# ecml-peagnn/graph_recsys_benchmark

Hardware: AMD Instinct MI355X
Metric: BPR-scored edges/sec, PEAGAT MovieLens-25m, emb_dim=64, 9 metapaths (higher is better)
Workload: dtype f32; 1 GPU; ml25m_shaped PEAGAT forward+BPR: N=273744 nodes, 9 metapaths x 2 steps, 208376439 messages/step, emb 64 / hidden 64 / repr 16, batch 4096 triples; headline=True, parallelism=single

## Files before the change

graph_recsys_benchmark_amd/csrc/ablate.hip:

```cpp
#include <algorithm>

#include "model.h"
#include "score_common.h"

namespace pea {
namespace {

template <int G, int PREG>
__global__ __launch_bounds__(256) void fuse_ablate_kernel(int64_t N, int P, int R, const float *__restrict__ stack,
                                                          int64_t ld, const ChanCols col_of_channel,
                                                          const float *__restrict__ att, int mode,
                                                          float *__restrict__ out, float *__restrict__ out_att) {
    const int64_t item = (int64_t)blockIdx.x * (256 / G) + threadIdx.x / G;
    const int sl = threadIdx.x % G;
    const bool valid = item < N;
    const int64_t n = valid ? item : 0;
    const bool in_row = sl * 4 < R;
    const bool active = valid && in_row;
    const int c4 = in_row ? sl * 4 : 0;
    const float *row = stack + n * ld + c4;
    const float4 zero = make_float4(0.f, 0.f, 0.f, 0.f);
    const bool mean = mode == PEA_FUSE_MEAN;
    float *dst = out + n * R + c4;
    const int64_t variant_stride = N * (int64_t)R;

    if constexpr (PREG > 0) {
        float4 x[PREG];
        float lg[PREG];
#pragma unroll
        for (int p = 0; p < PREG; ++p) {
            x[p] = zero;
            lg[p] = 0.f;
            if (p < P) {
                x[p] = ld4(row + col_of_channel.c[p]);
                if (!mean) lg[p] = chan_logit<G>(x[p], ld4(att + p * R + c4), in_row);
            }
        }
        for (int v = 0; v <= P; ++v) {
            const int masked = v - 1;
            float m = -3.0e38f, s = 0.f;
            float4 acc = zero;
#pragma unroll
            for (int p = 0; p < PREG; ++p) {
                if (p < P) {
                    const bool off = p == masked;
                    const float4 xv = off ? zero : x[p];
                    if (mean) {
                        acc.x += xv.x; acc.y += xv.y; acc.z += xv.z; acc.w += xv.w;
                    } else {
                        softmax_step(off ? 0.f : lg[p], xv, m, s, acc);
                    }
                }
            }
            const float inv = mean ? 1.0f / (float)P : 1.0f / s;
            if (active)
                *reinterpret_cast<float4 *>(dst + (int64_t)v * variant_stride) =
                    make_float4(acc.x * inv, acc.y * inv, acc.z * inv, acc.w * inv);
            if (v == 0 && out_att && valid) {
#pragma unroll
                for (int p = 0; p < PREG; ++p)
                    if (p < P && p % G == sl) out_att[n * P + p] = mean ? inv : expf(lg[p] - m) * inv;
            }
        }
    } else {
        for (int v = 0; v <= P; ++v) {
            const int masked = v - 1;
            float m = -3.0e38f, s = 0.f;
            float4 acc = zero;
            for (int p = 0; p < P; ++p) {
                float4 xv = ld4(row + col_of_channel.c[p]);
                if (p == masked) xv = zero;
                if (mean) {
                    acc.x += xv.x; acc.y += xv.y; acc.z += xv.z; acc.w += xv.w;
                    continue;
                }
                softmax_step(chan_logit<G>(xv, ld4(att + p * R + c4), in_row), xv, m, s, acc);
            }
            const float inv = mean ? 1.0f / (float)P : 1.0f / s;
            if (active)
                *reinterpret_cast<float4 *>(dst + (int64_t)v * variant_stride) =
                    make_float4(acc.x * inv, acc.y * inv, acc.z * inv, acc.w * inv);
            if (v == 0 && out_att) {
                for (int p = 0; p < P; ++p) {
                    float w = inv;
                    if (!mean) w = expf(chan_logit<G>(ld4(row + col_of_channel.c[p]), ld4(att + p * R + c4), in_row) - m) * inv;
                    if (valid && p % G == sl) out_att[n * P + p] = w;
                }
            }
        }
    }
}

constexpr int kRegSmall = 4, kRegChannels = 16;

template <int G>
int launch_fuse_ablate_g(int64_t N, int P, int R, const float *stack, int64_t ld, const ChanCols &cols, const float *att,
                         int mode, float *out, float *out_att, hipStream_t stream) {
    const unsigned blocks = (unsigned)((N + (256 / G) - 1) / (256 / G));
    if (P <= kRegSmall)
        PEA_LAUNCH((fuse_ablate_kernel<G, kRegSmall>), dim3(blocks), dim3(256), 0, stream, N, P, R, stack, ld, cols, att, mode,
                   out, out_att);
    else if (P <= kRegChannels)
        PEA_LAUNCH((fuse_ablate_kernel<G, kRegChannels>), dim3(blocks), dim3(256), 0, stream, N, P, R, stack, ld, cols, att,
                   mode, out, out_att);
    else
        PEA_LAUNCH((fuse_ablate_kernel<G, 0>), dim3(blocks), dim3(256), 0, stream, N, P, R, stack, ld, cols, att, mode, out,
                   out_att);
    PEA_HIP(hipGetLastError());
    return PEA_OK;
}

}

int launch_fuse_ablate(int64_t N, int P, int R, const float *stack, int64_t ld, const ChanCols &col_of_channel,
                       const float *att, int mode, float *out_tables, float *out_att, hipStream_t stream) {
    PEA_REQUIRE(N > 0 && stack && out_tables, PEA_ERR_ARG, "fuse_ablate: null argument");
    PEA_REQUIRE(P > 0 && P <= kMaxChannels && R > 0 && R % 4 == 0 && R <= 256, PEA_ERR_ARG,
                "fuse_ablate: P=%d R=%d (P <= 64, R a multiple of 4 and <= 256)", P, R);
    PEA_REQUIRE(mode == PEA_FUSE_ATT || mode == PEA_FUSE_MEAN, PEA_ERR_ARG, "fuse_ablate: mode %d", mode);
    PEA_REQUIRE(mode == PEA_FUSE_MEAN || att != nullptr, PEA_ERR_ARG, "fuse_ablate: att is required for 'att' fusion");
    PEA_REQUIRE(ld % 4 == 0, PEA_ERR_ARG, "fuse_ablate: stack row stride must be a multiple of 4");
    ProfScope ps("fuse_ablate", stream, 4.0 * (double)N * R * (2.0 * P + 1.0));
    switch (lanes_for_r(R)) {
        case 1: return launch_fuse_ablate_g<1>(N, P, R, stack, ld, col_of_channel, att, mode, out_tables, out_att, stream);
        case 2: return launch_fuse_ablate_g<2>(N, P, R, stack, ld, col_of_channel, att, mode, out_tables, out_att, stream);
        case 4: return launch_fuse_ablate_g<4>(N, P, R, stack, ld, col_of_channel, att, mode, out_tables, out_att, stream);
        case 8: return launch_fuse_ablate_g<8>(N, P, R, stack, ld, col_of_channel, att, mode, out_tables, out_att, stream);
        case 16: return launch_fuse_ablate_g<16>(N, P, R, stack, ld, col_of_channel, att, mode, out_tables, out_att, stream);
        case 32: return launch_fuse_ablate_g<32>(N, P, R, stack, ld, col_of_channel, att, mode, out_tables, out_att, stream);
        default: return launch_fuse_ablate_g<64>(N, P, R, stack, ld, col_of_channel, att, mode, out_tables, out_att, stream);
    }
}

}

using namespace pea;

extern "C" int pea_fuse_ablate(int64_t num_nodes, int P, int R, const float *stack, int64_t ld_stack,
                               const int *col_of_channel_host, const float *att, int fuse_mode, float *out_tables,
                               float *out_att, void *stream) {
    PEA_REQUIRE(num_nodes > 0 && stack && out_tables && col_of_channel_host, PEA_ERR_ARG, "fuse_ablate: null argument");
    PEA_REQUIRE(P > 0 && P <= kMaxChannels, PEA_ERR_ARG, "fuse_ablate: P=%d (1..%d)", P, kMaxChannels);
    ChanCols cols{};
    for (int p = 0; p < P; ++p) {
        PEA_REQUIRE(col_of_channel_host[p] >= 0 && col_of_channel_host[p] % 4 == 0 && col_of_channel_host[p] + R <= ld_stack,
                    PEA_ERR_ARG, "fuse_ablate: channel %d column %d outside the stack row", p, col_of_channel_host[p]);
        cols.c[p] = col_of_channel_host[p];
    }
    return launch_fuse_ablate(num_nodes, P, R, stack, ld_stack, cols, att, fuse_mode, out_tables, out_att, (hipStream_t)stream);
}

extern "C" int pea_model_forward_ablate(pea_model *model, const float *const *params_host, const float *x, const float *att,
                                        void *workspace, size_t workspace_bytes, float *out_tables, float *out_att,
                                        void *stream) {
    PEA_REQUIRE(out_tables, PEA_ERR_ARG, "forward_ablate: null argument");
    PEA_REQUIRE(!model || model->plan->shard_world == 1, PEA_ERR_ARG, "forward_ablate: single GPU only (the plan is sharded)");
    PEA_TRY(check_forward_args("forward_ablate", model, params_host, x, workspace, workspace_bytes, -1, nullptr));
    PEA_REQUIRE(model->d.fuse_mode == PEA_FUSE_MEAN || att, PEA_ERR_ARG, "forward_ablate: att is required for 'att' fusion");
    const AblateOut abl{out_tables, out_att};
    ForwardCall c;
    c.model = model;
    c.params = params_host;
    c.x = x;
    c.ldx = model->d.emb_dim;
    c.att = att;
    c.wsf = aligned_ws(workspace);
    c.stream = (hipStream_t)stream;
    c.abl = &abl;
    return model_forward(c);
}
```

graph_recsys_benchmark_amd/csrc/common.h:

```cpp
#pragma once
#include <hip/hip_runtime.h>

#include <cstdarg>
#include <cstdint>
#include <cstdio>
#include <functional>
#include <string>
#include <vector>

#include "../../include/peahip.h"

namespace pea {

void set_error(const char *fmt, ...);
const char *get_error();

#define PEA_HIP(call)                                                                          \
    do {                                                                                       \
        hipError_t e_ = (call);                                                                \
        if (e_ != hipSuccess) {                                                                \
            pea::set_error("%s:%d: %s failed: %s", __FILE__, __LINE__, #call,                 \
                           hipGetErrorString(e_));                                             \
            return PEA_ERR_HIP;                                                                \
        }                                                                                      \
// ... 293 lines not shown
    int blk_start[kMaxMlp2Chan + 1];
    const float *x;
    const float *a0;
    float *t1;
    float *images;
    float *bias1, *att_src1, *att_dst1;
    float *r1;
    int64_t ld_r1;
    int64_t ldx, ld_a0, ld_t1;
    float *h0;
    int64_t ld_h0;
    Mlp2Chan c[kMaxMlp2Chan];
};
size_t mlp2_image_bytes(int kind, int emb, int hid);
bool mlp2_supported(int kind, int emb, int hid, int out);
int launch_mlp2_pack(const Mlp2Launch &L, hipStream_t stream);
int launch_mlp2(const Mlp2Launch &L, const int *rows, int64_t n_rows, hipStream_t stream);

constexpr int kMaxChannels = 64;
constexpr int kScatterMaxCols = 1024;
struct ChanCols {
    int c[kMaxChannels];
};
struct FuseSelect {
    const int64_t *ids = nullptr;
    int64_t id_stride = 1, n = 0;
    float *out = nullptr;
    int *err = nullptr;
    int rank = 0, world = 1, tile = 1;
};
int launch_fuse(int64_t N, int P, int R, const float *stack, int64_t ld, const ChanCols &col_of_channel,
                const float *att, int masked, int mode, const int *rows, int64_t n_rows, float *out,
                float *out_stack, hipStream_t stream, const FuseSelect *sel = nullptr);

int launch_fuse_ablate(int64_t N, int P, int R, const float *stack, int64_t ld, const ChanCols &col_of_channel,
                       const float *att, int mode, float *out_tables, float *out_att, hipStream_t stream);
struct AblateOut {
    float *tables = nullptr;
    float *att = nullptr;
};

struct ForwardCall {
    pea_model *model = nullptr;
    int stage = -1;
    int part = PEA_PART_ALL;
    const float *const *params = nullptr;
    const float *x = nullptr;
    int64_t ldx = 0;
    const float *att = nullptr;
    int masked = -1;
    float *wsf = nullptr;
    float *out_repr = nullptr, *out_stack = nullptr;
    float *out_x = nullptr;
    int64_t ld_out_x = 0;
    int relu_last = 0;
    hipStream_t stream = nullptr;
    bool training = false;
    const FuseSelect *sel = nullptr;
    const AblateOut *abl = nullptr;
// ... 9 lines not shown
```

graph_recsys_benchmark_amd/csrc/fuse_score.hip:

```cpp
#include <algorithm>
#include <mutex>

#include "score_common.h"

namespace pea {
namespace {

template <int G>
__global__ __launch_bounds__(256) void fuse_kernel(int64_t n_rows, const int *__restrict__ rows, int P, int R,
                                                   const float *__restrict__ stack, int64_t ld,
                                                   const ChanCols col_of_channel,
                                                   const float *__restrict__ att, int masked, int mode,
                                                   float *__restrict__ out, float *__restrict__ out_stack,
                                                   unsigned fuse_blocks, const FuseSelect sel, int64_t N) {
    const bool pick = blockIdx.x >= fuse_blocks;
    const int64_t item = (int64_t)(pick ? blockIdx.x - fuse_blocks : blockIdx.x) * (256 / G) + threadIdx.x / G;
    const int sl = threadIdx.x % G;
    bool valid = item < (pick ? sel.n : n_rows);
    int64_t n = 0;
    if (pick) {
        const int64_t id = valid ? sel.ids[item * sel.id_stride] : 0;
        const bool in_range = id >= 0 && id < N;
        if (valid && !in_range && sl == 0) atomicOr(sel.err, 1);
        const bool mine = in_range && (id / sel.tile) % sel.world == sel.rank;
        if (valid && !mine && sl * 4 < R) *reinterpret_cast<float4 *>(sel.out + item * R + sl * 4) = make_float4(0.f, 0.f, 0.f, 0.f);
        valid = valid && mine;
        n = valid ? id : 0;
        out_stack = nullptr;
    } else {
        n = valid ? (rows ? rows[item] : item) : 0;
    }
    float *dst_row = pick ? sel.out + item * R : (out ? out + n * R : nullptr);
    const bool active = valid && sl * 4 < R;
    const int c4 = sl * 4 < R ? sl * 4 : 0;
    float m = -3.0e38f, s = 0.f;
    float4 acc = make_float4(0.f, 0.f, 0.f, 0.f);
    for (int p = 0; p < P; ++p) {
        float4 x = ld4(stack + n * ld + col_of_channel.c[p] + c4);
        if (p == masked) x = make_float4(0.f, 0.f, 0.f, 0.f);
        if (out_stack && active) *reinterpret_cast<float4 *>(out_stack + (n * P + p) * R + c4) = x;
        if (mode == PEA_FUSE_MEAN) {
            acc.x += x.x; acc.y += x.y; acc.z += x.z; acc.w += x.w;
            continue;
        }
        softmax_step(chan_logit<G>(x, ld4(att + p * R + c4), sl * 4 < R), x, m, s, acc);
    }
    if (!active || !dst_row) return;
    const float inv = mode == PEA_FUSE_MEAN ? 1.0f / (float)P : 1.0f / s;
    *reinterpret_cast<float4 *>(dst_row + c4) = make_float4(acc.x * inv, acc.y * inv, acc.z * inv, acc.w * inv);
}

__global__ __launch_bounds__(256) void bpr_kernel(int64_t B, int R, int64_t N, const float *__restrict__ repr,
                                                  const int64_t *__restrict__ triples, int64_t stride,
                                                  const float *fc1_w, const float *fc1_b, const float *fc2_w,
                                                  const float *fc2_b, float *pos, float *neg, float *block_sums,
                                                  int *err) {
    stage_mlp(R, fc1_w, fc1_b, fc2_w);
    const float *w1 = smem, *b1 = smem + 2 * R * R, *w2 = b1 + R;
    __shared__ float red[256];
    const int64_t b = (int64_t)blockIdx.x * 256 + threadIdx.x;
    float term = 0.f;
// ... 78 lines not shown
    if (uidx >= U) return;
    const int64_t u = unids[uidx];
    if (u < 0 || u >= N) {
        if (lane == 0) atomicOr(err, 1);
        return;
    }
    const bool shared = cand_stride == 0;
    int64_t keep0 = -1, keep1 = -1;
    if (shared) {
        if (lane < C) keep0 = cand[uidx * C + lane];
        if (kWave + lane < C) keep1 = cand[uidx * C + kWave + lane];
    }
    const float b2 = fc2_b[0];
    for (int v = 0; v < V; ++v) {
        const int64_t *cv = cand + (int64_t)v * cand_stride + uidx * C;
        const MlpScorer score(tables + (int64_t)v * N * R, u, R, b2);
        rank_one_user(score, [&](int base, int c) { return shared && base == 0 ? keep0 : shared && base == kWave ? keep1 : cv[c]; },
                      C, N, lane, (int64_t)v * U + uidx, scores, rank, auc, loss, err);
    }
}

}

int launch_fuse(int64_t N, int P, int R, const float *stack, int64_t ld, const ChanCols &col_of_channel,
                const float *att, int masked, int mode, const int *rows, int64_t n_rows, float *out,
                float *out_stack, hipStream_t stream, const FuseSelect *sel_in) {
    PEA_REQUIRE(P > 0 && P <= kMaxChannels && R > 0 && R % 4 == 0 && R <= 256, PEA_ERR_ARG,
                "fuse: P=%d R=%d (P <= 64, R a multiple of 4 and <= 256)", P, R);
    PEA_REQUIRE(masked < P, PEA_ERR_ARG, "fuse: masked channel %d out of range (P=%d)", masked, P);
    PEA_REQUIRE(mode == PEA_FUSE_MEAN || att != nullptr, PEA_ERR_ARG, "fuse: att is required for 'att' fusion");
    PEA_REQUIRE(ld % 4 == 0, PEA_ERR_ARG, "fuse: stack row stride must be a multiple of 4");
    if (!rows) n_rows = N;
    FuseSelect sel;
    if (sel_in && sel_in->n > 0) {
        sel = *sel_in;
        PEA_REQUIRE(sel.ids && sel.out && sel.err && sel.world >= 1 && sel.tile >= 1 && out != nullptr, PEA_ERR_ARG,
                    "fuse: batch-row selection needs ids, an output, an error flag and the fused table");
    }
    if (n_rows <= 0 && sel.n <= 0) return PEA_OK;
    const int G = lanes_for_r(R);
    ProfScope ps("fuse", stream, 4.0 * (double)(n_rows + sel.n) * R * (P + 1));
    const unsigned fuse_blocks = (unsigned)((std::max<int64_t>(n_rows, 0) + (256 / G) - 1) / (256 / G));
    const unsigned blocks = fuse_blocks + (unsigned)((sel.n + (256 / G) - 1) / (256 / G));
#define PEA_FUSE_CASE(g)                                                                                       \
    case g:                                                                                                    \
        PEA_LAUNCH(fuse_kernel<g>, dim3(blocks), dim3(256), 0, stream, n_rows, rows, P, R, stack, ld, \
                           col_of_channel, att, masked, mode, out, out_stack, fuse_blocks, sel, N);            \
        break;
    switch (G) {
        PEA_FUSE_CASE(1)
        PEA_FUSE_CASE(2)
        PEA_FUSE_CASE(4)
        PEA_FUSE_CASE(8)
        PEA_FUSE_CASE(16)
        PEA_FUSE_CASE(32)
        default:
            PEA_LAUNCH(fuse_kernel<64>, dim3(blocks), dim3(256), 0, stream, n_rows, rows, P, R, stack, ld,
                               col_of_channel, att, masked, mode, out, out_stack, fuse_blocks, sel, N);
    }
#undef PEA_FUSE_CASE
    PEA_HIP(hipGetLastError());
    return PEA_OK;
}

}

using pea::set_error;
using pea::err_flag_for_current_device;
using pea::read_err_flag;

extern "C" size_t pea_bpr_workspace_bytes(int64_t B) {
    const int64_t blocks = (B + 255) / 256;
    return (size_t)(blocks + 1) * sizeof(float) + 16;
}

static int check_r(int R) {
    PEA_REQUIRE(R > 0 && R % 4 == 0 && R <= 64, PEA_ERR_ARG, "repr_dim %d must be a multiple of 4, <= 64", R);
    return PEA_OK;
}

int *pea::err_flag_for_current_device() {
// ... 95 lines not shown
    {
        pea::ProfScope ps("rank_eval_multi", stream, (double)V * U * C * (4.0 * R + 12.0));
        PEA_LAUNCH(pea::rank_multi_kernel, dim3((unsigned)((U + 3) / 4)), dim3(256), sh, stream, V, U, C, R, num_nodes, tables, unids,
                   cand, cand_variant_stride, fc1_w, fc1_b, fc2_w, fc2_b, scores, rank, auc, loss, err);
    }
    int rc = hipGetLastError() == hipSuccess ? PEA_OK : PEA_ERR_HIP;
    if (rc == PEA_OK) rc = read_err_flag(err, stream, "rank_eval_multi");
    return rc;
}

extern "C" int pea_fuse(int64_t num_nodes, int P, int R, const float *stack, int64_t ld_stack,
                        const int *col_of_channel_host, const float *att, int masked_channel, int fuse_mode, float *out,
                        void *stream) {
    PEA_REQUIRE(num_nodes > 0 && stack && out && col_of_channel_host, PEA_ERR_ARG, "fuse: null argument");
    PEA_REQUIRE(P > 0 && P <= pea::kMaxChannels, PEA_ERR_ARG, "fuse: P=%d (1..%d)", P, pea::kMaxChannels);
    PEA_REQUIRE(fuse_mode == PEA_FUSE_ATT || fuse_mode == PEA_FUSE_MEAN, PEA_ERR_ARG, "fuse: mode %d", fuse_mode);
    PEA_REQUIRE(masked_channel >= -1, PEA_ERR_ARG, "fuse: masked channel %d", masked_channel);
    pea::ChanCols cols{};
    for (int p = 0; p < P; ++p) {
        PEA_REQUIRE(col_of_channel_host[p] >= 0 && col_of_channel_host[p] % 4 == 0 && col_of_channel_host[p] + R <= ld_stack,
                    PEA_ERR_ARG, "fuse: channel %d column %d outside the stack row", p, col_of_channel_host[p]);
        cols.c[p] = col_of_channel_host[p];
    }
    return pea::launch_fuse(num_nodes, P, R, stack, ld_stack, cols, att, masked_channel, fuse_mode, nullptr, num_nodes, out,
                            nullptr, (hipStream_t)stream);
}
```

graph_recsys_benchmark_amd/csrc/mlp2.hip:

```cpp
#include "common.h"

namespace pea {
namespace {

typedef float f32x16 __attribute__((ext_vector_type(16)));

__host__ __device__ inline int mlp2_image_floats(int ET, int HT) { return HT * ET * 256 + HT * 1024 + 2 * HT * 16; }

__global__ __launch_bounds__(256) void mlp2_pack_kernel(const Mlp2Launch L) {
    const int kPackSplit = (int)gridDim.x / L.n;
    const int chan = (int)blockIdx.x / kPackSplit, part = (int)blockIdx.x % kPackSplit;
    const Mlp2Chan &C = L.c[chan];
    const int EMB = L.emb, HID = L.hid, OUT = L.out;
    const int ET = EMB / 8, HT = HID / 32;
    const int t0 = part * 256 + (int)threadIdx.x, ts = 256 * kPackSplit;
    if (L.kind == PEA_KIND_SAGE) {
        const int KT = 2 * ET;
        float *img = L.images + (size_t)chan * mlp2_image_floats(KT, HT);
        float *wt0 = img, *wt1 = img + HT * KT * 256, *b0p = wt1 + HT * 1024;
        for (int idx = t0; idx < HT * KT * 256; idx += ts) {
            const int e = idx & 3, lane = (idx >> 2) & 63, qq = (idx >> 8) % KT, t = (idx >> 8) / KT;
            const int i = 32 * t + (lane & 31), k = 4 * (2 * (qq % ET) + (lane >> 5)) + e;
            wt0[idx] = (qq < ET ? C.w0 : C.w0_root)[(size_t)i * EMB + k];
        }
// ... 12 lines not shown
    float *img = L.images + (size_t)chan * mlp2_image_floats(ET, HT);
    float *wt0 = img, *wt1 = img + HT * ET * 256, *b0p = wt1 + HT * 1024;
    const bool gat = L.kind == PEA_KIND_GAT;
    const int EJ = EMB / 16, HJ = HID / 16;
    for (int idx = t0; idx < HJ * EJ * 256; idx += ts) {
        const int e = idx & 3, lane = (idx >> 2) & 63, j = (idx >> 8) % EJ, t = (idx >> 8) / EJ;
        const int i = 16 * t + (lane & 15), k = 16 * j + 4 * (lane >> 4) + e;
        wt0[idx] = gat ? C.w0[(size_t)i * EMB + k] : C.w0[(size_t)k * HID + i];
    }
    for (int idx = t0; idx < 2 * HJ * 256; idx += ts) {
        const int v = idx & 3, lane = (idx >> 2) & 63, t = (idx >> 8) % HJ, u = (idx >> 8) / HJ;
        const int o = 16 * u + (lane & 15), i = 16 * t + 4 * (lane >> 4) + v;
        wt1[idx] = o < OUT ? (gat ? C.w1[(size_t)o * HID + i] : C.w1[(size_t)i * OUT + o]) : 0.f;
    }
    for (int i = t0; i < HID; i += ts) b0p[i] = C.b0 ? C.b0[i] : 0.f;
    for (int o = t0; o < OUT; o += ts) {
        L.bias1[C.t1_col + o] = C.b1 ? C.b1[o] : 0.f;
        if (gat) {
            L.att_src1[C.t1_col + o] = C.att_src1[o];
            L.att_dst1[C.t1_col + o] = C.att_dst1[o];
        }
    }
    if (gat) {
        for (int k = (int)threadIdx.x * kPackSplit + part; k < EMB; k += ts) {
            float s = 0.f, d = 0.f;
            for (int i = 0; i < HID; ++i) {
                const float w = C.w0[(size_t)i * EMB + k];
                s = fmaf(C.att_src0[i], w, s);
                d = fmaf(C.att_dst0[i], w, d);
            }
            C.ws[k] = s;
            C.wd[k] = d;
        }
    }
}

extern __shared__ float mlp2_lds[];
template <int ET, int HT>
struct Mlp2Cfg {
    static constexpr int kThreads = (ET == 8 && HT == 2) ? 1024 : 512;
};

template <int ET>
struct Mlp2In {
    float4 xa[2][ET / 2];
    float sc[2];
    int row[2];
    bool valid[2];
};

template <int ET>
__device__ __forceinline__ void mlp2_load(const Mlp2Launch &L, const int *rows, int64_t n_rows, int64_t tile, int ch, int n16,
// ... 400 lines not shown
```

graph_recsys_benchmark_amd/csrc/model.hip:

```cpp
#include <algorithm>
#include <cstdlib>
#include <cstring>

#include "agg_build.h"

namespace pea {
namespace {

int pad4(int v) { return (v + 3) & ~3; }
int pad_ld(int v) { return (v + 31) & ~31; }
size_t pad_off(size_t v) { return (v + 63) & ~(size_t)63; }

int width_out(const pea_model_desc &d, int S, int s, int *heads_out) {
    const bool last = s == S - 1;
    int heads = d.kind == PEA_KIND_GAT ? d.heads : 1;
    if (S > 1 && last) heads = 1;
    *heads_out = heads;
    return last ? d.repr_dim : d.hidden_size;
}

int slots_of(const pea_model *m, int rel) {
    int n = m->plan->rels[(size_t)rel].n_slots;
    if (m->backward && rel < (int)m->reverse_of.size() && m->reverse_of[(size_t)rel] >= 0)
        n = std::max(n, m->plan->rels[(size_t)m->reverse_of[(size_t)rel]].n_slots);
// ... 334 lines not shown
    if (m->backward) {
        PEA_REQUIRE(desc->reverse_of != nullptr, PEA_ERR_ARG, "model: enable_backward needs reverse_of (relation -> reversed relation)");
        m->reverse_of.assign(desc->reverse_of, desc->reverse_of + plan->rels.size());
    }
    m->d.steps = nullptr;
    m->d.relation_of = nullptr;
    m->d.reverse_of = nullptr;
    m->n_slots_per_layer = desc->kind == PEA_KIND_GAT ? 4 : desc->kind == PEA_KIND_GCN ? 2 : 3;
    return build_schedule(m);
}

struct Fwd {
    const ForwardCall &c;
    pea_model *m;
    pea_plan *plan;
    float *pack;
    float *X;
    int64_t ldX;
    float *partial;
    bool sharded;
    const int *own_rows;
    int64_t n_own;
    bool hot_on;

    explicit Fwd(const ForwardCall &call)
        : c(call), m(call.model), plan(const_cast<pea_plan *>(call.model->plan)), pack(call.wsf),
          X(call.out_x ? call.out_x : call.wsf + call.model->off_x), ldX(call.out_x ? call.ld_out_x : call.model->ld_x),
          partial(call.wsf + call.model->off_partial), sharded(plan->shard_world > 1),
          own_rows(sharded ? plan->owned_rows : nullptr), n_own(sharded ? plan->n_owned : plan->N) {
        const char *hot_env = getenv("PEA_HOT");
        hot_on = hot_env && atoi(hot_env) != 0;
    }
    const float *param(const Unit &u, int slot) const {
        return c.params[(size_t)(m->chan_first[(size_t)u.p] + u.s) * (size_t)m->n_slots_per_layer + (size_t)slot];
    }
    bool self_loops() const { return (plan->flags & PEA_PLAN_SELF_LOOPS) != 0; }
};

struct LevelIO {
    Level &L;
    float *T, *O;
    const float *In;
    int ldIn;
    LevelOut out;
};
LevelIO level_io(const Fwd &f, int s) {
    pea_model *m = f.m;
    Level &L = m->levels[(size_t)s];
    float *O = f.c.wsf + L.off_o;
    return LevelIO{L,
                   f.c.wsf + L.off_t,
                   O,
                   s == 0 ? f.c.x : f.c.wsf + m->levels[(size_t)s - 1].off_o,
                   s == 0 ? (int)f.c.ldx : m->levels[(size_t)s - 1].ld_o,
// ... 64 lines not shown
        a.hot_K = hv->K;
        a.hot_frac = R.e_kept > 0 ? (double)hv->hot_edges / (double)R.e_kept : 0.0;
    }
    return PEA_OK;
}

AggMode forward_mode(int kind) { return kind == PEA_KIND_GAT ? AGG_GAT : kind == PEA_KIND_GCN ? AGG_GCN : AGG_MEAN; }

int aggregate_level(const Fwd &f, int s, AggMode mode) {
    const pea_model *m = f.m;
    pea_plan *plan = f.plan;
    const pea_model_desc &d = m->d;
    const bool training = f.c.training;
    float *wsf = f.c.wsf;
    const LevelIO io = level_io(f, s);
    const Level &L = io.L;
    const bool via_slots = f.sharded && s > 0;
    const bool mean2 = mode == AGG_MEAN && m->sage2;
    std::vector<AggGroup> gs;
    for (const GroupPlan &g : L.groups) {
        Relation &R = plan->rels[(size_t)g.rel];
        if (via_slots) PEA_REQUIRE(R.col_slot != nullptr, PEA_ERR_ARG, "relation %d has no exchange layout (pea_plan_set_sources)", g.rel);
        AggGroup a = agg_over(R);
        const bool skip0 = mode != AGG_MEAN && !g.last && f.self_loops() && !training;
        const bool skip0_mean = mean2 && !g.last && !training;
        if (skip0 || skip0_mean) skip_edgeless(a, R);
        if (training && mode == AGG_GAT) {
            a.stats = wsf + L.off_stats + 2 * g.a_k;
            a.ld_stats = L.ld_stats;
        }
        a.W = g.W;
        a.F = g.F;
        a.partial = f.partial + g.partial_off;
        a.neg_slope = d.negative_slope;
        set_traffic(a, R, mode != AGG_MEAN && f.self_loops() ? 1.0 : 0.0, mode == AGG_MEAN ? 1.0 : (double)g.n_convs,
                    table_rows(R, plan, via_slots));
        const Dest out = io.out.at(g.last, g.out_col);
        if (mode == AGG_MEAN && !mean2) {
            a.feat = io.In + g.col;
            a.ld_feat = io.ldIn;
            a.out = io.T + g.out_col;
            a.ld_out = L.ld_t;
        } else {
            a.feat = io.T + g.col;
            a.ld_feat = L.ld_t;
            a.out = out.ptr;
            a.ld_out = out.ld;
// ... 130 lines not shown
        GemmJob J = gemm_job(io.In, io.ldIn, f.m->d.emb_dim, f.pack + L.b_off + c_beg, L.ldb, c_end - c_beg, c_end - c_beg,
                             io.T + c_beg, L.ld_t);
        J.no_narrow = 1;
        J.rows = R.need_rows;
        J.n_rows = R.n_need;
        jobs.push_back(J);
        i = j;
    }
    root_jobs(f, 0, jobs);
    return launch_gemm_batch(jobs.data(), (int)jobs.size(), nullptr, 0, f.c.stream);
}

int transform_units(const Fwd &f, int s) {
    const LevelIO io = level_io(f, s);
    std::vector<GemmJob> jobs;
    for (const Unit &u : io.L.units) {
        GemmJob J = gemm_job(io.In + u.in_col, io.ldIn, u.in_w, f.pack + u.b_off, u.ldb, u.ldb, u.HF, io.T + u.t_col, io.L.ld_t);
        if (f.m->sage2 && !f.c.training) relu_on_load(f, s, u, J);
        if (f.self_loops() && !f.c.training) PEA_TRY(conv_on_load(f, s, u, J));
        jobs.push_back(J);
    }
    root_jobs(f, s, jobs);
    return launch_gemm_batch(jobs.data(), (int)jobs.size(), f.own_rows, f.n_own, f.c.stream);
}

int transform_level(const Fwd &f, int s) {
    if (f.m->d.kind == PEA_KIND_SAGE && !f.m->sage2) return transform_mean_first(f, s);
    if (!f.m->levels[(size_t)s].shared_input) return transform_units(f, s);
    return f.sharded ? transform_shared_sharded(f) : transform_shared(f);
}


int set_exchange(const Fwd &f, const Unit &u1, Mlp2Chan &C) {
    C.x_slot = nullptr;
    C.x_buf = nullptr;
    C.x_ld = 0;
    if (!f.sharded) return PEA_OK;
    for (const GroupPlan &g : f.m->levels[1].groups) {
        if (u1.t_col < g.col || u1.t_col >= g.col + g.W) continue;
        const Relation &R2 = f.plan->rels[(size_t)g.rel];
        PEA_REQUIRE(R2.slot_of_node != nullptr && g.xch_ld > 0, PEA_ERR_ARG,
                    "relation %d has no exchange layout (pea_plan_set_sources)", g.rel);
        C.x_slot = R2.slot_of_node;
        C.x_buf = f.c.wsf + g.xch_off + (u1.t_col - g.col);
        C.x_ld = g.xch_ld;
        return PEA_OK;
// ... 137 lines not shown
    const pea_model_desc &d = m->d;
    const int n_levels = (int)m->levels.size();
    const Fwd f(c);
    if (f.sharded) PEA_REQUIRE(f.plan->owned_rows != nullptr || f.plan->n_owned == 0, PEA_ERR_ARG, "sharded plan without owned rows");
    const int s_beg = c.stage < 0 ? 0 : c.stage, s_end = c.stage < 0 ? n_levels : c.stage + 1;
    PEA_REQUIRE(s_beg >= 0 && s_end <= n_levels, PEA_ERR_ARG, "forward: stage %d of %d", c.stage, n_levels);
    PEA_REQUIRE(c.part == PEA_PART_ALL || (f.sharded && c.stage >= 0), PEA_ERR_ARG, "forward: parts are stages of a sharded plan");
    const bool splits = m->fused2 && !c.training;
    const bool two_step = (m->fused2 && !c.training) || (m->fused2_train && c.training);
    const bool mean_first = d.kind == PEA_KIND_SAGE && !m->sage2;
    const AggMode mode = forward_mode(d.kind);
    for (int k = s_beg; k < s_end; ++k) {
        if (c.part == PEA_PART_REST && !(splits && k == 0)) continue;
        if (two_step) {
            PEA_TRY(k == 0 ? two_step_stage0(f) : aggregate_level(f, k, mode));
        } else {
            if (k == 0) PEA_TRY(pack_weights(f));
            if (k == 0 && !mean_first) PEA_TRY(transform_level(f, 0));
            PEA_TRY(aggregate_level(f, k, mode));
            if (mean_first) PEA_TRY(transform_level(f, k));
            else if (k + 1 < n_levels) PEA_TRY(transform_level(f, k + 1));
        }
        if (k != n_levels - 1) continue;
        if (c.abl)
            PEA_TRY(launch_fuse_ablate(f.plan->N, d.num_channels, d.repr_dim, f.X, f.ldX, m->x_col, c.att, d.fuse_mode, c.abl->tables,
                                       c.abl->att, c.stream));
        else if (c.out_repr || c.out_stack)
            PEA_TRY(launch_fuse(f.plan->N, d.num_channels, d.repr_dim, f.X, f.ldX, m->x_col, c.att, c.masked, d.fuse_mode, f.own_rows,
                                f.n_own, c.out_repr, c.out_stack, c.stream, c.sel));
    }
    return PEA_OK;
}

int check_forward_args(const char *who, const pea_model *model, const float *const *params, const float *x,
                       const void *workspace, size_t workspace_bytes, int masked, const int *stage) {
    PEA_REQUIRE(model && params && x && workspace, PEA_ERR_ARG, "%s: null argument", who);
    const int n_stages = (int)model->levels.size();
    if (stage) PEA_REQUIRE(*stage >= 0 && *stage < n_stages, PEA_ERR_ARG, "%s: stage %d of %d", who, *stage, n_stages);
    PEA_REQUIRE(workspace_bytes >= pea_model_workspace_bytes(model), PEA_ERR_NOMEM, "%s: workspace %zu < %zu bytes", who,
                workspace_bytes, pea_model_workspace_bytes(model));
    PEA_REQUIRE(masked >= -1 && masked < model->d.num_channels, PEA_ERR_ARG, "%s: masked channel %d", who, masked);
    return PEA_OK;
}

}

using namespace pea;

extern "C" int pea_model_create(const pea_plan *plan, const pea_model_desc *desc, pea_model **out) {
    PEA_REQUIRE(out != nullptr, PEA_ERR_ARG, "model: out is null");
    *out = nullptr;
    pea_model *m = new pea_model();
// ... 219 lines not shown
```

graph_recsys_benchmark_amd/csrc/score_common.h:

```cpp
#ifndef PEA_SCORE_COMMON_H_
#define PEA_SCORE_COMMON_H_

#include "common.h"

namespace pea {

int *err_flag_for_current_device();
int read_err_flag(int *err_dev, hipStream_t stream, const char *what);

inline int lanes_for_r(int R) {
    int g = 1;
    while (g * 4 < R) g <<= 1;
    return g;
}

namespace {

__device__ __forceinline__ float mlp_score(const float *__restrict__ ur, const float *__restrict__ ir, int R,
                                           const float *w1, const float *b1, const float *w2, float b2) {
    float o = 0.f;
    for (int k = 0; k < R; ++k) {
        const float *w = w1 + k * 2 * R;
        float a = 0.f;
        for (int c = 0; c < R; c += 4) {
            const float4 u = ld4(ur + c), wu = ld4(w + c);
            a += (u.x * wu.x + u.y * wu.y) + (u.z * wu.z + u.w * wu.w);
// ... 27 lines not shown
            a += (v[c].x * wi.x + v[c].y * wi.y) + (v[c].z * wi.z + v[c].w * wi.w);
        }
        a += b1[k];
        o = fmaf(fmaxf(a, 0.f), w2[k], o);
    }
    return o + b2;
}

template <int R4>
__device__ __forceinline__ void load_row(const float *p, float4 (&r)[R4]) {
#pragma unroll
    for (int c = 0; c < R4; ++c) r[c] = ld4(p + 4 * c);
}

extern __shared__ float smem[];

__device__ __forceinline__ void stage_mlp(int R, const float *fc1_w, const float *fc1_b, const float *fc2_w) {
    for (int i = threadIdx.x; i < 2 * R * R; i += blockDim.x) smem[i] = fc1_w[i];
    for (int i = threadIdx.x; i < R; i += blockDim.x) {
        smem[2 * R * R + i] = fc1_b[i];
        smem[2 * R * R + R + i] = fc2_w[i];
    }
    __syncthreads();
}

__device__ __forceinline__ float log_sigmoid_ref(float d) {
    return logf(1.0f / (1.0f + expf(-d)));
}

struct MlpScorer {
    const float *repr, *w1, *b1, *w2;
    float b2;
    int R;
    int64_t u;
    float4 ur[4];
    __device__ __forceinline__ MlpScorer(const float *repr_, int64_t u_, int R_, float b2_)
        : repr(repr_), w1(smem), b1(smem + 2 * R_ * R_), w2(smem + 2 * R_ * R_ + R_), b2(b2_), R(R_), u(u_) {
        if (R == 16) load_row<4>(repr + u * R, ur);
    }
    __device__ __forceinline__ float operator()(int64_t i) const {
        if (R == 16) {
            float4 ir[4];
            load_row<4>(repr + i * R, ir);
            return mlp_score_reg<4>(ur, ir, w1, b1, w2, b2);
        }
        return mlp_score(repr + u * R, repr + i * R, R, w1, b1, w2, b2);
// ... 66 lines not shown
```

Baseline: 129.7 billion edges/s.

## Defer edgeless-node last-layer rows to fuse kernel via self-loop copy path

For inference forwards that end in a fuse or ablate step, the last aggregation level now also skips edgeless (degree-zero) nodes. Their output is rebuilt inside the fuse kernels from the transformed row, bias, attention or GCN normalisation, and ReLU, with bias and attention vectors staged in LDS. This avoids a separate aggregation pass over those rows at the cost of more per-channel work and branching in the fuse kernels and extra LDS use. The GAT weight-folding loop in mlp2 is also unrolled into batched loads.

```diff
diff --git a/graph_recsys_benchmark_amd/csrc/ablate.hip b/graph_recsys_benchmark_amd/csrc/ablate.hip
--- a/graph_recsys_benchmark_amd/csrc/ablate.hip
+++ b/graph_recsys_benchmark_amd/csrc/ablate.hip
@@ -8,7 +8,7 @@
 
 template <int G, int PREG>
 __global__ __launch_bounds__(256) void fuse_ablate_kernel(int64_t N, int P, int R, const float *__restrict__ stack,
-                                                          int64_t ld, const ChanCols col_of_channel,
+                                                          int64_t ld, const ChanCols col_of_channel, const ChanCopy copy,
                                                           const float *__restrict__ att, int mode,
                                                           float *__restrict__ out, float *__restrict__ out_att) {
     const int64_t item = (int64_t)blockIdx.x * (256 / G) + threadIdx.x / G;
@@ -18,11 +18,13 @@
     const bool in_row = sl * 4 < R;
     const bool active = valid && in_row;
     const int c4 = in_row ? sl * 4 : 0;
-    const float *row = stack + n * ld + c4;
+    const float *row0 = stack + n * ld;
     const float4 zero = make_float4(0.f, 0.f, 0.f, 0.f);
     const bool mean = mode == PEA_FUSE_MEAN;
     float *dst = out + n * R + c4;
     const int64_t variant_stride = N * (int64_t)R;
+    const unsigned long long lone = copy_row_bits(copy, P, n);
+    stage_copy_rows(copy, P, R, smem);
 
     if constexpr (PREG > 0) {
         float4 x[PREG];
@@ -32,7 +34,7 @@
             x[p] = zero;
             lg[p] = 0.f;
             if (p < P) {
-                x[p] = ld4(row + col_of_channel.c[p]);
+                x[p] = chan_value(row0 + col_of_channel.c[p], copy.c[p], copy, smem + 3 * p * R, R, (lone >> p) & 1, n, c4, sl);
                 if (!mean) lg[p] = chan_logit<G>(x[p], ld4(att + p * R + c4), in_row);
             }
         }
@@ -68,7 +70,7 @@
             float m = -3.0e38f, s = 0.f;
             float4 acc = zero;
             for (int p = 0; p < P; ++p) {
-                float4 xv = ld4(row + col_of_channel.c[p]);
+                float4 xv = chan_value(row0 + col_of_channel.c[p], copy.c[p], copy, smem + 3 * p * R, R, (lone >> p) & 1, n, c4, sl);
                 if (p == masked) xv = zero;
                 if (mean) {
                     acc.x += xv.x; acc.y += xv.y; acc.z += xv.z; acc.w += xv.w;
@@ -83,7 +85,7 @@
             if (v == 0 && out_att) {
                 for (int p = 0; p < P; ++p) {
                     float w = inv;
-                    if (!mean) w = expf(chan_logit<G>(ld4(row + col_of_channel.c[p]), ld4(att + p * R + c4), in_row) - m) * inv;
+                    if (!mean) w = expf(chan_logit<G>(chan_value(row0 + col_of_channel.c[p], copy.c[p], copy, smem + 3 * p * R, R, (lone >> p) & 1, n, c4, sl), ld4(att + p * R + c4), in_row) - m) * inv;
                     if (valid && p % G == sl) out_att[n * P + p] = w;
                 }
             }
@@ -94,18 +96,18 @@
 constexpr int kRegSmall = 4, kRegChannels = 16;
 
 template <int G>
-int launch_fuse_ablate_g(int64_t N, int P, int R, const float *stack, int64_t ld, const ChanCols &cols, const float *att,
+int launch_fuse_ablate_g(int64_t N, int P, int R, const float *stack, int64_t ld, const ChanCols &cols, const ChanCopy &copy, const float *att,
                          int mode, float *out, float *out_att, hipStream_t stream) {
     const unsigned blocks = (unsigned)((N + (256 / G) - 1) / (256 / G));
     if (P <= kRegSmall)
-        PEA_LAUNCH((fuse_ablate_kernel<G, kRegSmall>), dim3(blocks), dim3(256), 0, stream, N, P, R, stack, ld, cols, att, mode,
-                   out, out_att);
+        PEA_LAUNCH((fuse_ablate_kernel<G, kRegSmall>), dim3(blocks), dim3(256), copy_lds_bytes(copy, P, R), stream, N, P, R, stack, ld, cols, copy, att,
+                   mode, out, out_att);
     else if (P <= kRegChannels)
-        PEA_LAUNCH((fuse_ablate_kernel<G, kRegChannels>), dim3(blocks), dim3(256), 0, stream, N, P, R, stack, ld, cols, att,
+        PEA_LAUNCH((fuse_ablate_kernel<G, kRegChannels>), dim3(blocks), dim3(256), copy_lds_bytes(copy, P, R), stream, N, P, R, stack, ld, cols, copy, att,
                    mode, out, out_att);
     else
-        PEA_LAUNCH((fuse_ablate_kernel<G, 0>), dim3(blocks), dim3(256), 0, stream, N, P, R, stack, ld, cols, att, mode, out,
-                   out_att);
+        PEA_LAUNCH((fuse_ablate_kernel<G, 0>), dim3(blocks), dim3(256), copy_lds_bytes(copy, P, R), stream, N, P, R, stack, ld, cols, copy, att, mode,
+                   out, out_att);
     PEA_HIP(hipGetLastError());
     return PEA_OK;
 }
@@ -113,22 +115,23 @@
 }
 
 int launch_fuse_ablate(int64_t N, int P, int R, const float *stack, int64_t ld, const ChanCols &col_of_channel,
-                       const float *att, int mode, float *out_tables, float *out_att, hipStream_t stream) {
+                       const ChanCopy &copy, const float *att, int mode, float *out_tables, float *out_att, hipStream_t stream) {
     PEA_REQUIRE(N > 0 && stack && out_tables, PEA_ERR_ARG, "fuse_ablate: null argument");
     PEA_REQUIRE(P > 0 && P <= kMaxChannels && R > 0 && R % 4 == 0 && R <= 256, PEA_ERR_ARG,
                 "fuse_ablate: P=%d R=%d (P <= 64, R a multiple of 4 and <= 256)", P, R);
     PEA_REQUIRE(mode == PEA_FUSE_ATT || mode == PEA_FUSE_MEAN, PEA_ERR_ARG, "fuse_ablate: mode %d", mode);
     PEA_REQUIRE(mode == PEA_FUSE_MEAN || att != nullptr, PEA_ERR_ARG, "fuse_ablate: att is required for 'att' fusion");
     PEA_REQUIRE(ld % 4 == 0, PEA_ERR_ARG, "fuse_ablate: stack row stride must be a multiple of 4");
+    PEA_REQUIRE(copy_lds_bytes(copy, P, R) <= kCopyLdsMax, PEA_ERR_ARG, "fuse_ablate: copy rows of a %d x %d stack", P, R);
     ProfScope ps("fuse_ablate", stream, 4.0 * (double)N * R * (2.0 * P + 1.0));
     switch (lanes_for_r(R)) {
-        case 1: return launch_fuse_ablate_g<1>(N, P, R, stack, ld, col_of_channel, att, mode, out_tables, out_att, stream);
-        case 2: return launch_fuse_ablate_g<2>(N, P, R, stack, ld, col_of_channel, att, mode, out_tables, out_att, stream);
-        case 4: return launch_fuse_ablate_g<4>(N, P, R, stack, ld, col_of_channel, att, mode, out_tables, out_att, stream);
-        case 8: return launch_fuse_ablate_g<8>(N, P, R, stack, ld, col_of_channel, att, mode, out_tables, out_att, stream);
-        case 16: return launch_fuse_ablate_g<16>(N, P, R, stack, ld, col_of_channel, att, mode, out_tables, out_att, stream);
-        case 32: return launch_fuse_ablate_g<32>(N, P, R, stack, ld, col_of_channel, att, mode, out_tables, out_att, stream);
-        default: return launch_fuse_ablate_g<64>(N, P, R, stack, ld, col_of_channel, att, mode, out_tables, out_att, stream);
+        case 1: return launch_fuse_ablate_g<1>(N, P, R, stack, ld, col_of_channel, copy, att, mode, out_tables, out_att, stream);
+        case 2: return launch_fuse_ablate_g<2>(N, P, R, stack, ld, col_of_channel, copy, att, mode, out_tables, out_att, stream);
+        case 4: return launch_fuse_ablate_g<4>(N, P, R, stack, ld, col_of_channel, copy, att, mode, out_tables, out_att, stream);
+        case 8: return launch_fuse_ablate_g<8>(N, P, R, stack, ld, col_of_channel, copy, att, mode, out_tables, out_att, stream);
+        case 16: return launch_fuse_ablate_g<16>(N, P, R, stack, ld, col_of_channel, copy, att, mode, out_tables, out_att, stream);
+        case 32: return launch_fuse_ablate_g<32>(N, P, R, stack, ld, col_of_channel, copy, att, mode, out_tables, out_att, stream);
+        default: return launch_fuse_ablate_g<64>(N, P, R, stack, ld, col_of_channel, copy, att, mode, out_tables, out_att, stream);
     }
 }
 
@@ -147,7 +150,7 @@
                     PEA_ERR_ARG, "fuse_ablate: channel %d column %d outside the stack row", p, col_of_channel_host[p]);
         cols.c[p] = col_of_channel_host[p];
     }
-    return launch_fuse_ablate(num_nodes, P, R, stack, ld_stack, cols, att, fuse_mode, out_tables, out_att, (hipStream_t)stream);
+    return launch_fuse_ablate(num_nodes, P, R, stack, ld_stack, cols, ChanCopy{}, att, fuse_mode, out_tables, out_att, (hipStream_t)stream);
 }
 
 extern "C" int pea_model_forward_ablate(pea_model *model, const float *const *params_host, const float *x, const float *att,
diff --git a/graph_recsys_benchmark_amd/csrc/common.h b/graph_recsys_benchmark_amd/csrc/common.h
--- a/graph_recsys_benchmark_amd/csrc/common.h
+++ b/graph_recsys_benchmark_amd/csrc/common.h
@@ -339,6 +339,23 @@
 struct ChanCols {
     int c[kMaxChannels];
 };
+struct CopyRows {
+    const unsigned char *deg0;
+    const float *t;
+    const float *bias;
+    const float *dinv;
+    int ld;
+    int F;
+    int att_src_at, att_dst_at;
+};
+struct ChanCopy {
+    int on = 0;
+    int relu = 0;
+    float neg_slope = 0.f;
+    CopyRows c[kMaxChannels] = {};
+};
+inline size_t copy_lds_bytes(const ChanCopy &cc, int P, int R) { return cc.on ? (size_t)3 * P * R * sizeof(float) : 0; }
+constexpr size_t kCopyLdsMax = 48 * 1024;
 struct FuseSelect {
     const int64_t *ids = nullptr;
     int64_t id_stride = 1, n = 0;
@@ -346,12 +363,12 @@
     int *err = nullptr;
     int rank = 0, world = 1, tile = 1;
 };
-int launch_fuse(int64_t N, int P, int R, const float *stack, int64_t ld, const ChanCols &col_of_channel,
+int launch_fuse(int64_t N, int P, int R, const float *stack, int64_t ld, const ChanCols &col_of_channel, const ChanCopy &copy,
                 const float *att, int masked, int mode, const int *rows, int64_t n_rows, float *out,
                 float *out_stack, hipStream_t stream, const FuseSelect *sel = nullptr);
 
 int launch_fuse_ablate(int64_t N, int P, int R, const float *stack, int64_t ld, const ChanCols &col_of_channel,
-                       const float *att, int mode, float *out_tables, float *out_att, hipStream_t stream);
+                       const ChanCopy &copy, const float *att, int mode, float *out_tables, float *out_att, hipStream_t stream);
 struct AblateOut {
     float *tables = nullptr;
     float *att = nullptr;
diff --git a/graph_recsys_benchmark_amd/csrc/fuse_score.hip b/graph_recsys_benchmark_amd/csrc/fuse_score.hip
--- a/graph_recsys_benchmark_amd/csrc/fuse_score.hip
+++ b/graph_recsys_benchmark_amd/csrc/fuse_score.hip
@@ -9,7 +9,7 @@
 template <int G>
 __global__ __launch_bounds__(256) void fuse_kernel(int64_t n_rows, const int *__restrict__ rows, int P, int R,
                                                    const float *__restrict__ stack, int64_t ld,
-                                                   const ChanCols col_of_channel,
+                                                   const ChanCols col_of_channel, const ChanCopy copy,
                                                    const float *__restrict__ att, int masked, int mode,
                                                    float *__restrict__ out, float *__restrict__ out_stack,
                                                    unsigned fuse_blocks, const FuseSelect sel, int64_t N) {
@@ -35,8 +35,10 @@
     const int c4 = sl * 4 < R ? sl * 4 : 0;
     float m = -3.0e38f, s = 0.f;
     float4 acc = make_float4(0.f, 0.f, 0.f, 0.f);
+    const unsigned long long lone = copy_row_bits(copy, P, n);
+    stage_copy_rows(copy, P, R, smem);
     for (int p = 0; p < P; ++p) {
-        float4 x = ld4(stack + n * ld + col_of_channel.c[p] + c4);
+        float4 x = chan_value(stack + n * ld + col_of_channel.c[p], copy.c[p], copy, smem + 3 * p * R, R, (lone >> p) & 1, n, c4, sl);
         if (p == masked) x = make_float4(0.f, 0.f, 0.f, 0.f);
         if (out_stack && active) *reinterpret_cast<float4 *>(out_stack + (n * P + p) * R + c4) = x;
         if (mode == PEA_FUSE_MEAN) {
@@ -161,7 +163,7 @@
 
 }
 
-int launch_fuse(int64_t N, int P, int R, const float *stack, int64_t ld, const ChanCols &col_of_channel,
+int launch_fuse(int64_t N, int P, int R, const float *stack, int64_t ld, const ChanCols &col_of_channel, const ChanCopy &copy,
                 const float *att, int masked, int mode, const int *rows, int64_t n_rows, float *out,
                 float *out_stack, hipStream_t stream, const FuseSelect *sel_in) {
     PEA_REQUIRE(P > 0 && P <= kMaxChannels && R > 0 && R % 4 == 0 && R <= 256, PEA_ERR_ARG,
@@ -178,13 +180,15 @@
     }
     if (n_rows <= 0 && sel.n <= 0) return PEA_OK;
     const int G = lanes_for_r(R);
+    const size_t lds = copy_lds_bytes(copy, P, R);
+    PEA_REQUIRE(lds <= kCopyLdsMax, PEA_ERR_ARG, "fuse: copy rows of a %d x %d stack", P, R);
     ProfScope ps("fuse", stream, 4.0 * (double)(n_rows + sel.n) * R * (P + 1));
     const unsigned fuse_blocks = (unsigned)((std::max<int64_t>(n_rows, 0) + (256 / G) - 1) / (256 / G));
     const unsigned blocks = fuse_blocks + (unsigned)((sel.n + (256 / G) - 1) / (256 / G));
 #define PEA_FUSE_CASE(g)                                                                                       \
     case g:                                                                                                    \
-        PEA_LAUNCH(fuse_kernel<g>, dim3(blocks), dim3(256), 0, stream, n_rows, rows, P, R, stack, ld, \
-                           col_of_channel, att, masked, mode, out, out_stack, fuse_blocks, sel, N);            \
+        PEA_LAUNCH(fuse_kernel<g>, dim3(blocks), dim3(256), lds, stream, n_rows, rows, P, R, stack, ld, \
+                           col_of_channel, copy, att, masked, mode, out, out_stack, fuse_blocks, sel, N);            \
         break;
     switch (G) {
         PEA_FUSE_CASE(1)
@@ -194,8 +198,8 @@
         PEA_FUSE_CASE(16)
         PEA_FUSE_CASE(32)
         default:
-            PEA_LAUNCH(fuse_kernel<64>, dim3(blocks), dim3(256), 0, stream, n_rows, rows, P, R, stack, ld,
-                               col_of_channel, att, masked, mode, out, out_stack, fuse_blocks, sel, N);
+            PEA_LAUNCH(fuse_kernel<64>, dim3(blocks), dim3(256), lds, stream, n_rows, rows, P, R, stack, ld,
+                               col_of_channel, copy, att, masked, mode, out, out_stack, fuse_blocks, sel, N);
     }
 #undef PEA_FUSE_CASE
     PEA_HIP(hipGetLastError());
@@ -337,6 +341,6 @@
                     PEA_ERR_ARG, "fuse: channel %d column %d outside the stack row", p, col_of_channel_host[p]);
         cols.c[p] = col_of_channel_host[p];
     }
-    return pea::launch_fuse(num_nodes, P, R, stack, ld_stack, cols, att, masked_channel, fuse_mode, nullptr, num_nodes, out,
+    return pea::launch_fuse(num_nodes, P, R, stack, ld_stack, cols, pea::ChanCopy{}, att, masked_channel, fuse_mode, nullptr, num_nodes, out,
                             nullptr, (hipStream_t)stream);
 }
diff --git a/graph_recsys_benchmark_amd/csrc/mlp2.hip b/graph_recsys_benchmark_amd/csrc/mlp2.hip
--- a/graph_recsys_benchmark_amd/csrc/mlp2.hip
+++ b/graph_recsys_benchmark_amd/csrc/mlp2.hip
@@ -58,12 +58,25 @@
         }
     }
     if (gat) {
+        constexpr int kPackTerms = 16;
         for (int k = (int)threadIdx.x * kPackSplit + part; k < EMB; k += ts) {
             float s = 0.f, d = 0.f;
-            for (int i = 0; i < HID; ++i) {
-                const float w = C.w0[(size_t)i * EMB + k];
-                s = fmaf(C.att_src0[i], w, s);
-                d = fmaf(C.att_dst0[i], w, d);
+            for (int i0 = 0; i0 < HID; i0 += kPackTerms) {
+                float w[kPackTerms], as[kPackTerms], ad[kPackTerms];
+#pragma unroll
+                for (int u = 0; u < kPackTerms; ++u) {
+                    const int i = min(i0 + u, HID - 1);
+                    w[u] = C.w0[(size_t)i * EMB + k];
+                    as[u] = C.att_src0[i];
+                    ad[u] = C.att_dst0[i];
+                }
+#pragma unroll
+                for (int u = 0; u < kPackTerms; ++u) {
+                    if (i0 + u < HID) {
+                        s = fmaf(as[u], w[u], s);
+                        d = fmaf(ad[u], w[u], d);
+                    }
+                }
             }
             C.ws[k] = s;
             C.wd[k] = d;
diff --git a/graph_recsys_benchmark_amd/csrc/model.hip b/graph_recsys_benchmark_amd/csrc/model.hip
--- a/graph_recsys_benchmark_amd/csrc/model.hip
+++ b/graph_recsys_benchmark_amd/csrc/model.hip
@@ -380,6 +380,7 @@
     const int *own_rows;
     int64_t n_own;
     bool hot_on;
+    bool copy_at_fuse;
 
     explicit Fwd(const ForwardCall &call)
         : c(call), m(call.model), plan(const_cast<pea_plan *>(call.model->plan)), pack(call.wsf),
@@ -388,6 +389,10 @@
           own_rows(sharded ? plan->owned_rows : nullptr), n_own(sharded ? plan->n_owned : plan->N) {
         const char *hot_env = getenv("PEA_HOT");
         hot_on = hot_env && atoi(hot_env) != 0;
+        const char *visit_env = getenv("PEA_LAST_COPY_ROWS");
+        copy_at_fuse = !call.training && !call.out_x && (call.abl || call.out_repr || call.out_stack) &&
+                       m->d.kind != PEA_KIND_SAGE && self_loops() && !(visit_env && atoi(visit_env) != 0) &&
+                       (size_t)12 * m->d.num_channels * m->d.repr_dim <= kCopyLdsMax;
     }
     const float *param(const Unit &u, int slot) const {
         return c.params[(size_t)(m->chan_first[(size_t)u.p] + u.s) * (size_t)m->n_slots_per_layer + (size_t)slot];
@@ -498,7 +503,7 @@
         Relation &R = plan->rels[(size_t)g.rel];
         if (via_slots) PEA_REQUIRE(R.col_slot != nullptr, PEA_ERR_ARG, "relation %d has no exchange layout (pea_plan_set_sources)", g.rel);
         AggGroup a = agg_over(R);
-        const bool skip0 = mode != AGG_MEAN && !g.last && f.self_loops() && !training;
+        const bool skip0 = mode != AGG_MEAN && f.self_loops() && !training && (!g.last || f.copy_at_fuse);
         const bool skip0_mean = mean2 && !g.last && !training;
         if (skip0 || skip0_mean) skip_edgeless(a, R);
         if (training && mode == AGG_GAT) {
@@ -675,6 +680,35 @@
     }
     root_jobs(f, s, jobs);
     return launch_gemm_batch(jobs.data(), (int)jobs.size(), f.own_rows, f.n_own, f.c.stream);
+}
+
+int copy_rows_of(const Fwd &f, ChanCopy &cc) {
+    cc = ChanCopy{};
+    if (!f.copy_at_fuse) return PEA_OK;
+    cc.on = 1;
+    cc.relu = f.c.relu_last;
+    cc.neg_slope = f.m->d.negative_slope;
+    for (const Level &L : f.m->levels) {
+        for (const Unit &u : L.units) {
+            if (!u.last) continue;
+            Relation &R = f.plan->rels[(size_t)u.rel];
+            CopyRows &S = cc.c[u.p];
+            S.deg0 = R.deg0;
+            S.t = f.c.wsf + L.off_t + u.t_col;
+            S.ld = L.ld_t;
+            S.bias = f.pack + L.bias_off + u.t_col;
+            if (f.m->d.kind == PEA_KIND_GAT) {
+                S.F = u.F;
+                S.att_src_at = (int)(L.att_src_off - L.bias_off);
+                S.att_dst_at = (int)(L.att_dst_off - L.bias_off);
+            } else {
+                const bool fc = f.m->d.gcn_deg_from_col != 0;
+                PEA_TRY(ensure_dinv(f.plan, u.rel, fc, f.c.stream));
+                S.dinv = fc ? R.dinv_col : R.dinv_row;
+            }
+        }
+    }
+    return PEA_OK;
 }
 
 int transform_level(const Fwd &f, int s) {
@@ -858,12 +892,14 @@
             else if (k + 1 < n_levels) PEA_TRY(transform_level(f, k + 1));
         }
         if (k != n_levels - 1) continue;
+        ChanCopy copy;
+        PEA_TRY(copy_rows_of(f, copy));
         if (c.abl)
-            PEA_TRY(launch_fuse_ablate(f.plan->N, d.num_channels, d.repr_dim, f.X, f.ldX, m->x_col, c.att, d.fuse_mode, c.abl->tables,
-                                       c.abl->att, c.stream));
+            PEA_TRY(launch_fuse_ablate(f.plan->N, d.num_channels, d.repr_dim, f.X, f.ldX, m->x_col, copy, c.att, d.fuse_mode,
+                                       c.abl->tables, c.abl->att, c.stream));
         else if (c.out_repr || c.out_stack)
-            PEA_TRY(launch_fuse(f.plan->N, d.num_channels, d.repr_dim, f.X, f.ldX, m->x_col, c.att, c.masked, d.fuse_mode, f.own_rows,
-                                f.n_own, c.out_repr, c.out_stack, c.stream, c.sel));
+            PEA_TRY(launch_fuse(f.plan->N, d.num_channels, d.repr_dim, f.X, f.ldX, m->x_col, copy, c.att, c.masked, d.fuse_mode,
+                                f.own_rows, f.n_own, c.out_repr, c.out_stack, c.stream, c.sel));
     }
     return PEA_OK;
 }
diff --git a/graph_recsys_benchmark_amd/csrc/score_common.h b/graph_recsys_benchmark_amd/csrc/score_common.h
--- a/graph_recsys_benchmark_amd/csrc/score_common.h
+++ b/graph_recsys_benchmark_amd/csrc/score_common.h
@@ -1,7 +1,7 @@
 #ifndef PEA_SCORE_COMMON_H_
 #define PEA_SCORE_COMMON_H_
 
-#include "common.h"
+#include "agg_common.h"
 
 namespace pea {
 
@@ -75,6 +75,52 @@
         smem[2 * R * R + R + i] = fc2_w[i];
     }
     __syncthreads();
+}
+
+__device__ __forceinline__ unsigned long long copy_row_bits(const ChanCopy &cc, int P, int64_t n) {
+    unsigned long long bits = 0;
+    if (!cc.on) return bits;
+#pragma unroll 8
+    for (int p = 0; p < P; ++p) {
+        const unsigned char *flag = cc.c[p].deg0;
+        bits |= (unsigned long long)(flag != nullptr && flag[n] != 0) << p;
+    }
+    return bits;
+}
+
+__device__ __forceinline__ void stage_copy_rows(const ChanCopy &cc, int P, int R, float *lds) {
+    if (!cc.on) return;
+    for (int i = threadIdx.x; i < 3 * P * R; i += blockDim.x) {
+        const int c = i % R, k = (i / R) % 3;
+        const CopyRows &S = cc.c[i / (3 * R)];
+        float v = 0.f;
+        if (S.deg0 && (k == 0 || S.att_src_at)) v = S.bias[(k == 0 ? 0 : k == 1 ? S.att_src_at : S.att_dst_at) + c];
+        lds[i] = v;
+    }
+    __syncthreads();
+}
+
+__device__ __forceinline__ float4 chan_value(const float *row, const CopyRows &S, const ChanCopy &cc, const float *rows, int R,
+                                             bool lone, int64_t n, int c4, int sl) {
+    float4 v = ld4(lone ? S.t + n * S.ld + c4 : row + c4);
+    if (lone) {
+        if (S.dinv) {
+            const float di = S.dinv[n];
+            v = fma4(di * di, v, make_float4(0.f, 0.f, 0.f, 0.f));
+        } else if (S.att_src_at) {
+            const int lane = (int)threadIdx.x % kWave, F4 = S.F / 4, pos = sl % F4;
+            const bool pow2 = (F4 & (F4 - 1)) == 0;
+            const float a_d = head_sum<0>(dot4(v, ld4(rows + 2 * R + c4)), lane, pos, F4, pow2);
+            const float a = head_sum<0>(dot4(v, ld4(rows + R + c4)), lane, pos, F4, pow2);
+            Soft st;
+            st.init();
+            st.push(leaky(a + a_d, cc.neg_slope), v);
+            v = scale4(st.acc, 1.0f / (st.s + 1e-16f));
+        }
+        v = add4(v, ld4(rows + c4));
+        if (cc.relu) v = make_float4(fmaxf(v.x, 0.f), fmaxf(v.y, 0.f), fmaxf(v.z, 0.f), fmaxf(v.w, 0.f));
+    }
+    return v;
 }
 
 __device__ __forceinline__ float log_sigmoid_ref(float d) {
```

After: 131.8 billion edges/s (median of 6 runs). 1.02x the previous value.
